# cerbos/cerbos

Measured on NVIDIA H100. Metric: checkresources_decisions_per_sec, higher is better.
Workload: dtype u64

## Files before the change

### cerbos_b200/csrc/cb_core.h

```cpp
#pragma once
#include <stdint.h>
#if !defined(__CUDACC_RTC__)
#include <math.h>
#endif

#include "cerbos_b200_format.h"

#if defined(__CUDACC__)
#define CB_HD __host__ __device__ __forceinline__
#define CB_HD_NOINLINE __host__ __device__ __noinline__
#else
#define CB_HD inline
#define CB_HD_NOINLINE
#endif

namespace cb {

struct alignas(16) U4 { uint32_t x, y, z, w; };

struct TableLayout {
    uint32_t off[CB_IMAGE_SECTIONS];
    uint32_t nV, nRP, nS, nP, nR, nAP, nT, n_slots, n_rows;
    uint32_t has_role_policies, has_parent_roles, has_principal_policies;
    uint32_t image_bytes;
    uint32_t uc_conds_off, uc_rows_off, uc_chain_off, n_uconds;
    uint32_t uc_n_rows;
    uint32_t uc_slots_off;
    uint32_t uc_deny_rows, uc_allow_rows;
    uint32_t theap_words;
    uint32_t uses_runtime;
};

struct TableView {
    const uint8_t *base;
    const TableLayout *L;
    template <typename T>
    CB_HD const T *sec(int id) const { return reinterpret_cast<const T *>(base + L->off[id]); }
    CB_HD const uint32_t *scope_parent() const { return sec<uint32_t>(CB_SEC_SCOPE_PARENT); }
    CB_HD const uint32_t *scope_flags() const { return sec<uint32_t>(CB_SEC_SCOPE_FLAGS); }
    CB_HD const uint32_t *res_block_map() const { return sec<uint32_t>(CB_SEC_RES_BLOCK_MAP); }
    CB_HD const uint8_t *res_exists() const { return sec<uint8_t>(CB_SEC_RES_EXISTS); }
    CB_HD const uint32_t *prin_block_map() const { return sec<uint32_t>(CB_SEC_PRIN_BLOCK_MAP); }
    CB_HD const uint8_t *prin_exists() const { return sec<uint8_t>(CB_SEC_PRIN_EXISTS); }
    CB_HD const uint32_t *prin_of_string() const { return sec<uint32_t>(CB_SEC_PRIN_OF_STRING); }
    CB_HD const cb_block *blocks() const { return sec<cb_block>(CB_SEC_BLOCKS); }
    CB_HD const cb_row *rows() const { return sec<cb_row>(CB_SEC_ROWS); }
    CB_HD const cb_cond *conds() const { return sec<cb_cond>(CB_SEC_CONDS); }
    CB_HD const cb_instr *code() const { return sec<cb_instr>(CB_SEC_CODE); }
    CB_HD const cb_const *consts() const { return sec<cb_const>(CB_SEC_CONSTS); }
    CB_HD const uint64_t *consts_v64() const { return sec<uint64_t>(CB_SEC_CONSTS_V64); }
    CB_HD const uint64_t *theap() const { return sec<uint64_t>(CB_SEC_THEAP); }
    CB_HD const uint32_t *str_off() const { return sec<uint32_t>(CB_SEC_STR_OFF); }
    CB_HD const uint8_t *str_bytes() const { return sec<uint8_t>(CB_SEC_STR_BYTES); }
    CB_HD const uint32_t *par_off() const { return sec<uint32_t>(CB_SEC_ROLE_PARENTS_OFF); }
    CB_HD const uint32_t *par_list() const { return sec<uint32_t>(CB_SEC_ROLE_PARENTS); }
    CB_HD const uint32_t *rp_off() const { return sec<uint32_t>(CB_SEC_ROLEPOL_OFF); }
    CB_HD const cb_rolepol_entry *rp_entries() const { return sec<cb_rolepol_entry>(CB_SEC_ROLEPOL_ENTRIES); }
    CB_HD const cb_rolepol_rule *rp_rules() const { return sec<cb_rolepol_rule>(CB_SEC_ROLEPOL_RULES); }
    CB_HD const uint32_t *rp_apats() const { return sec<uint32_t>(CB_SEC_ROLEPOL_APATS); }
    CB_HD const uint32_t *block_slots_off() const { return sec<uint32_t>(CB_SEC_BLOCK_SLOTS_OFF); }
    CB_HD const uint32_t *block_slots() const { return sec<uint32_t>(CB_SEC_BLOCK_SLOTS); }
    CB_HD const uint32_t *dr_off() const { return sec<uint32_t>(CB_SEC_DR_OFF); }
    CB_HD const uint32_t *dr_entries() const { return sec<uint32_t>(CB_SEC_DR_ENTRIES); }
    CB_HD const uint32_t *dr_parents() const { return sec<uint32_t>(CB_SEC_DR_PARENTS); }
    CB_HD const uint32_t *dr_name_str() const { return sec<uint32_t>(CB_SEC_DR_NAME_STR); }
    CB_HD const uint32_t *row_out() const { return sec<uint32_t>(CB_SEC_ROW_OUT); }
    CB_HD const cb_out_entry *out_entries() const { return sec<cb_out_entry>(CB_SEC_OUT_ENTRIES); }
    CB_HD const cb_cond *uconds() const { return reinterpret_cast<const cb_cond *>(base + L->uc_conds_off); }
    CB_HD const U4 *urows() const { return reinterpret_cast<const U4 *>(base + L->uc_rows_off); }
    CB_HD const uint32_t *uc_slots() const { return reinterpret_cast<const uint32_t *>(base + L->uc_slots_off); }
    CB_HD const U4 *uc_chain() const { return reinterpret_cast<const U4 *>(base + L->uc_chain_off); }
};

enum { CB_MAX_GATHER = 8 };
struct BatchView {
    const cb_hdr0 *hdr0;
    const cb_hdr1 *hdr1;
    const uint32_t *roles;
// ... 4413 lines not shown
    CB_HD UcRowsPacked at(uint32_t first) const { UcRowsPacked r = *this; if (by_slot) r.pk += first; else r.slots += first; return r; }
    CB_HD U4 get(uint32_t ri) const { return ld16(pk + ri); }
    CB_HD U4 slot(uint32_t j) const {
        if (by_slot) return ld16(pk + j);
        const uint32_t ri = ldg(slots + j);
        return uc_slot_record(ld16(pk + (ri != CB_NONE32 ? ri : 0u)), ri != CB_NONE32);
    }
};

struct CachedCols {
    const BatchView *b;
    uint64_t n;
    CB_HD U4 hdr0() const { return ldcol128(b->hdr0 + n); }
    CB_HD uint64_t hdr1() const { return ldcol64(reinterpret_cast<const uint64_t *>(b->hdr1 + n)); }
    CB_HD uint32_t role(uint32_t i) const { return ldcol32(b->roles + (uint64_t)i * b->stride + n); }
    CB_HD uint64_t slot(uint32_t v) const {
#if defined(__CUDA_ARCH__)
        uint64_t x;
        asm("ld.global.nc.u64 %0, [%1];" : "=l"(x) : "l"(b->slots + (uint64_t)v * b->stride + n));
        return x;
#else
        return b->slots[(uint64_t)v * b->stride + n];
#endif
    }
    CB_HD void prefetch_slot(uint32_t) const {}
    CB_HD bool staged() const { return true; }
    CB_HD uint32_t aset_k(uint32_t aset) const { return ldg(b->aset_k + aset); }
    CB_HD const uint64_t *row_am() const { return b->row_am; }
    CB_HD bool stage_result(uint32_t) const { return false; }
};

struct CondWord { uint64_t lo, hi; };
enum { CB_UC_FORM_MASK32 = 0, CB_UC_FORM_MASK64 = 1, CB_UC_FORM_INDEX = 2 };
constexpr uint32_t kUcUnrollRows = 16;
constexpr uint32_t kUcRowsOfLayout = ~0u;
struct GenericConds {
    static constexpr int kForm = CB_UC_FORM_MASK64;
    static constexpr uint32_t kDenyRows = kUcRowsOfLayout, kAllowRows = kUcRowsOfLayout;
    static constexpr uint32_t kListSlots = 0;
    template <typename Cols>
    CB_HD Cols load(const TableView, const BatchView &, const Cols &cols) const { return cols; }
    template <typename Cols>
    CB_HD CondWord operator()(const TableView t, const BatchView &b, const Cols &cols, uint32_t pid, uint64_t n, bool &slow) const {
        if (t.L->n_uconds > 63) { slow = true; CondWord w; w.lo = 1; w.hi = 0; return w; }
        uint64_t val = 1;
        for (uint32_t u = 1, nu = t.L->n_uconds; u <= nu; u++) {
            const U4 cd = ld16(t.uconds() + u);
            uint32_t r;
            if (cd.w) r = flat_dnf_inline(t, b, cols, pid, cd.z, cd.w);
            else r = 4u;
            slow |= (r & 4u) != 0;
            val |= (uint64_t)(r & 1u) << u;
        }
        CondWord w; w.lo = val; w.hi = 0;
        return w;
    }
};

CB_HD uint32_t cond_bit(const CondWord v, uint32_t u) { return (uint32_t)(((u & 64u) ? v.hi : v.lo) >> (u & 63u)) & 1u; }
template <typename RP, int kForm>
CB_HD uint32_t uc_row_pairs(const U4 r, const RP rp, const CondWord v, const uint32_t role_all, const uint32_t shift) {
    const uint32_t vlo = (uint32_t)v.lo, vhi = (uint32_t)(v.lo >> 32);
    const uint32_t miss = kForm == CB_UC_FORM_MASK32   ? r.y & ~vlo
                          : kForm == CB_UC_FORM_MASK64 ? (r.y & ~vlo) | (r.z & ~vhi)
                                                       : (cond_bit(v, r.y & 0xFFu) & cond_bit(v, (r.y >> 8) & 0xFFu)) ^ 1u;
    const uint32_t rc = miss ? 0u : (uint32_t)(rp >> shift) & role_all;
    return r.x * rc;
}
struct UcNoObserver {
    CB_HD void operator()(uint32_t, uint32_t, uint32_t, uint32_t, const CondWord &) const {}
};
template <uint32_t kDenyRows, uint32_t kAllowRows, typename RP, int kForm, typename Rows, typename Obs = UcNoObserver>
CB_HD uint32_t uc_walk(const TableView t, const Rows rows, const RP rp, const CondWord val, const uint32_t r0, const uint32_t bm_base,
                       const uint32_t role_all, uint32_t alive, Obs &&obs = Obs()) {
    constexpr bool kOfLayout = kDenyRows == kUcRowsOfLayout;
    const uint32_t n_deny = kOfLayout ? t.L->uc_deny_rows : kDenyRows, n_allow = kOfLayout ? t.L->uc_allow_rows : kAllowRows;
    const bool segments = n_deny + n_allow != 0;
    uint32_t allow_pairs = 0, level = 0;
    const U4 *chain = t.uc_chain() + bm_base;
    for (uint32_t s = r0; s != CB_NONE32 && alive;) {
        const U4 d = ld16(chain + s);
        uint32_t D = 0, A = 0;
        if (segments) {
            const Rows seg = rows.at(d.x);
            auto slot = [&](uint32_t j) { const U4 r = seg.slot(j); return uc_row_pairs<RP, kForm>(r, rp, val, role_all, r.w); };
#if defined(__CUDA_ARCH__)
#pragma unroll
#endif
            for (uint32_t j = 0; j < n_deny; j++) D |= slot(j);
#if defined(__CUDA_ARCH__)
#pragma unroll
#endif
            for (uint32_t j = 0; j < n_allow; j++) A |= slot(n_deny + j);
            D |= A & d.z;
            A &= d.y;
        } else {
#if defined(__CUDA_ARCH__)
#pragma unroll 4
#endif
            for (uint32_t ri = d.x; ri < d.z; ri++) {
                const U4 r = rows.get(ri);
                const uint32_t p = uc_row_pairs<RP, kForm>(r, rp, val, role_all, r.w & (sizeof(RP) * 8 - 1)), deny = (uint32_t)((int32_t)r.w >> 31);
                D |= p & deny;
                A |= p & ~deny;
            }
        }
        D &= alive;
        alive &= ~D;
        A &= alive;
        allow_pairs |= A;
        alive &= ~A;
        obs(level++, s, D, A, val);
        s = d.w;
    }
    return allow_pairs;
}

template <typename Cols, typename Rows, typename Conds = GenericConds>
// ... 90 lines not shown
    for (uint32_t i = 0; i < RC; i++) {
        const uint32_t rr = cols.role(i);
        gap |= pad && rr != CB_ROLE_PAD;
        pad |= rr == CB_ROLE_PAD;
        n_roles = rr != CB_ROLE_PAD ? i + 1 : n_roles;
        rp |= rr < t.L->nR ? 1ull << (rr * RCP + i) : 0ull;
        req_roles |= rr < t.L->nR ? 1ull << rr : 0ull;
    }
    if (pv != rv || gap) return true;
    const bool lenient = (b.flags & CB_BATCH_FLAG_LENIENT) != 0;
    const uint32_t r0 = chain_start(t, rscope, CB_SCOPE_FLAG_RESOURCE, lenient), p0 = chain_start(t, pscope, CB_SCOPE_FLAG_PRINCIPAL, lenient);
    const uint32_t bm_base = (rv * t.L->nRP + kc) * t.L->nS;
    bool exists = false;
    if (K != 0 && r0 != CB_NONE32 && rv != CB_NONE16 && kc != CB_KIND_NONE) {
        const uint32_t w = ld16(side + bm_base + r0).z;
        if ((w >> 8) > CB_MAX_CHAIN) return true;
        exists = (w & 1u) != 0;
    }
    const bool walk = exists && n_roles != 0;
    const uint32_t role_all = (1u << n_roles) - 1;
    uint32_t allow_pairs = 0, acc = 0;
    uint64_t edr = 0;
    UcMetaObserver ob;
    CondWord val; val.lo = 1; val.hi = 0;
    if (walk) {
        bool slow = false;
        val = conds(t, b, regs, pid, n, slow);
        if (slow) return true;
        const uint32_t amask = K * RC >= 32 ? b.stride_pattern : b.stride_pattern & ((1u << (K * RC)) - 1);
        const uint32_t alive0 = amask * role_all;
        const Rows arows = rows.aset(t, b, aset);
        if ((t.L->nR + 1) * RCP <= 32)
            allow_pairs = uc_walk<Conds::kDenyRows, Conds::kAllowRows, uint32_t, Conds::kForm>(t, arows, (uint32_t)rp | role_all << (t.L->nR * RCP), val, r0, bm_base, role_all, alive0, ob);
        else allow_pairs = uc_walk<Conds::kDenyRows, Conds::kAllowRows, uint64_t, Conds::kForm>(t, arows, rp | (uint64_t)role_all << (t.L->nR * RCP), val, r0, bm_base, role_all, alive0, ob);
        uint32_t need = 0;
        for (uint32_t k = 0; k < K; k++) {
            const uint32_t a = (allow_pairs >> (k * RC)) & role_all, lowest = a & (0u - a);
            need |= (lowest ? lowest | (lowest - 1) : role_all) << (k * RC);
            acc |= (a != 0 ? 1u : 0u) << k;
        }
        const uint32_t undecided = alive0 & ~(allow_pairs | ob.deny), last = ob.levels - 1;
        const uint32_t lv0 = ob.lv0 | ((last & 1u) ? undecided : 0u), lv1 = ob.lv1 | ((last & 2u) ? undecided : 0u), lv2 = ob.lv2 | ((last & 4u) ? undecided : 0u);
        uint32_t top = 0, cand = need;
        if (cand & lv2) { top |= 4u; cand &= lv2; }
        if (cand & lv1) { top |= 2u; cand &= lv1; }
        if (cand & lv0) top |= 1u;
        const U4 *chain = t.uc_chain() + bm_base;
        uint32_t s = r0;
        for (uint32_t l = 0; l <= top && s != CB_NONE32; l++) {
            const U4 m = ld16(side + bm_base + s);
            for (uint32_t e = m.x; e < m.y; e++) {
                const U4 dr = ld16(side + e);
                const bool hit = (dr.y >> 31) != 0 || ((((uint64_t)dr.w << 32) | dr.z) & req_roles) != 0;
                edr |= (uint64_t)(hit && cond_bit(val, dr.y & 0x7FFFFFFFu)) << dr.x;
            }
            s = ld16(chain + s).w;
        }
    }
    store_result(b, cols, n, nullptr, effects, K, acc);
    uint32_t *am = action_meta + n * (uint64_t)KM;
    const uint32_t none = walk ? 0xFFFFu | CB_META_SRC_RESOURCE_POLICY << 16 : 0xFFFFu;
    const U4 *chain = t.uc_chain() + bm_base;
    for (uint32_t k = 0; k < KM; k++) {
        uint32_t w = 0xFFFFu;
        if (k < K) {
            const uint32_t a = (allow_pairs >> (k * RC)) & role_all, d = (ob.deny >> (k * RC)) & role_all, c = a ? a : d;
            w = none;
            if (c) {
                uint32_t s = r0;
                for (uint32_t l = 0, lv = ob.level_of(k * RC + ctz32(c)); l < lv; l++) s = ld16(chain + s).w;
                w = (s & 0xFFFFu) | CB_META_SRC_RESOURCE_POLICY << 16;
            }
        }
        am[k] = w;
    }
    cb_request_meta rm;
    rm.principal_first_scope = (uint16_t)(p0 == CB_NONE32 ? 0xFFFFu : p0);
    rm.resource_first_scope = (uint16_t)(r0 == CB_NONE32 ? 0xFFFFu : r0);
    rm.flags = 0;
    rm.effective_derived_roles = edr;
    req_meta[n] = rm;
    return false;
}

#ifndef CB_LEAN_ONLY
CB_HD_NOINLINE void eval_request_general(const uint8_t *base, const TableLayout *L, const BatchView *b, uint64_t n, uint8_t *bitmap,
                                         uint8_t *effects, uint32_t *status) {
    TableView t; t.base = base; t.L = L;
    eval_request<uint64_t>(t, *b, n, bitmap, effects, status);
}

#endif

}
```

### cerbos_b200/csrc/cb_specialize.h

```cpp
#pragma once
#include <stdint.h>

#include <cstdio>
#include <cstring>
#include <map>
#include <string>
#include <vector>

#include "cerbos_b200_format.h"

namespace cbspec {

struct Limits {
    uint32_t max_shapes = 8;
    uint32_t max_items = 96;
};

inline std::string hex(uint32_t v) {
    char buf[16];
    snprintf(buf, sizeof buf, "0x%xu", v);
    return buf;
}
inline std::string hex64(uint64_t v) {
    char buf[32];
// ... 334 lines not shown
        if (I.op == CB_OP_CONST && i + 1 < code_len) {
            const uint32_t nx = P[i + 1].op;
            if (cond_level(nx)) literal = true;
            if ((nx == CB_OP_JF_KEEP || nx == CB_OP_JT_KEEP) && (e >= code_len || P[i + 1].ic > e)) literal = true;
        }
        if (literal) {
            if (I.ic >= n_consts || consts[4 * I.ic] != CB_T_BOOL) return "";
            st.push_back(consts[4 * I.ic + 2] ? "true" : "false");
            i++;
            continue;
        }
        if (e >= code_len) return "";
        std::vector<uint32_t> key;
        for (uint32_t k = i; k < e; k++) {
            const Ins &J = P[k];
            const bool j = is_jump(J.op);
            key.push_back(J.op | J.ia << 8 | (J.op == CB_OP_TERN ? (J.ib - i) : J.ib) << 16);
            key.push_back(j ? J.ic - i : J.ic);
        }
        auto it = at.ids.find(key);
        if (it == at.ids.end()) {
            if (at.slot_used.size() < n_slots) at.slot_used.resize(n_slots, false);
            uint32_t one = CB_NONE32;
            bool pid = false;
            const std::string body = atom_source(P, i, e, consts, n_consts, n_slots, at.slot_used, &one, &pid);
            if (body.empty()) return "";
            const uint32_t id = (uint32_t)at.src.size();
            at.only_slot.push_back(one);
            at.reads_pid.push_back(pid);
            at.src.push_back("template <typename Cols>\nCB_HD bool uc_atom_" + std::to_string(id) + "(Ctx &c, const Cols &cols) {\n" + body + "}\n");
            it = at.ids.emplace(key, id).first;
        }
        st.push_back("a" + std::to_string(it->second));
        i = e + 1;
    }
    if (!ret || st.size() != 1) return "";
    return st[0];
}

struct UcLimits {
    uint32_t max_terms = 512;
};
struct UcSource {
    std::string src;
    uint32_t n_strpred = 0;
    uint32_t n_atoms = 0;
};
inline UcSource generate_uc(const uint8_t *uc_image, const uint32_t *off, uint32_t uc_conds_off, uint32_t n_uconds, uint32_t n_slots, uint32_t n_consts = 0,
                            const UcLimits lim = UcLimits()) {
    UcSource out;
    if (n_uconds == 0 || n_uconds > 127) return out;
    const uint32_t *const_words = reinterpret_cast<const uint32_t *>(uc_image + off[CB_SEC_CONSTS]);
    Atoms atoms;
    std::vector<std::string> formula(n_uconds + 1);
    const uint32_t *uconds = reinterpret_cast<const uint32_t *>(uc_image + uc_conds_off);
    const uint32_t scope_rows = uconds[0], deny_rows = uconds[1], allow_rows = uconds[2];
    const uint32_t *code = reinterpret_cast<const uint32_t *>(uc_image + off[CB_SEC_CODE]);
    const uint64_t *consts = reinterpret_cast<const uint64_t *>(uc_image + off[CB_SEC_CONSTS_V64]);
    const uint64_t *theap = reinterpret_cast<const uint64_t *>(uc_image + off[CB_SEC_THEAP]);
    const uint32_t kUseMask = ~((uint32_t)(CB_TERM_LIT_F | CB_TERM_GROUP_END) << 8);
    std::map<std::vector<uint32_t>, uint32_t> term_ids;
    std::vector<std::vector<uint32_t>> terms;
    const uint32_t ns = n_slots ? n_slots : 1;
    std::vector<bool> slot_used(ns, false), slot_list(ns, false);
    auto is_slot_kind = [](uint32_t kind) { return kind == CB_OPK_SLOT || kind == CB_OPK_SLOT_ELEM || kind == CB_OPK_SLOT_SIZE; };
    auto use_slot = [&](uint32_t kind, uint32_t v) { if (is_slot_kind(kind) && v < ns) slot_used[v] = true; };
    auto v64_tag = [](uint64_t b) { const uint32_t top = (uint32_t)(b >> 48); return (top & 0xFFF0u) == 0xFFF0u ? (top & 0xFu) : 0u; };
    for (uint32_t u = 1; u <= n_uconds; u++) {
        const uint32_t *cd = uconds + 4 * u;
        if (cd[3] == 0 || ((cd[3] >> 16) & 0xFF) != CB_FLAT_DNF) {
            formula[u] = translate_program(code, cd[0], cd[1], const_words, n_consts, ns, atoms);
            if (formula[u].empty()) return out;
            continue;
        }
        for (uint32_t i = 0, nt = cd[3] & 0xFFFFu; i < nt; i++) {
            const uint32_t *w = code + 2 * (cd[2] + 2 * i);
            std::vector<uint32_t> key = {w[0] & kUseMask, w[1], w[2], w[3]};
            if (term_ids.emplace(key, (uint32_t)terms.size()).second) terms.push_back(key);
        }
    }
    if (terms.size() > lim.max_terms) return out;
    std::vector<char> form(terms.size(), 'G');
    std::vector<uint32_t> pred_of(terms.size(), 0);
    std::vector<uint32_t> pred_terms;
    for (uint32_t q = 0; q < terms.size(); q++) {
        const uint32_t *w = terms[q].data();
        const uint32_t op = w[0] & 0xFF, xk = (w[0] >> 16) & 0xFF, yk = w[0] >> 24;
        switch (op) {
        case CB_TERM_EQ_SS: case CB_TERM_ORD_SS: use_slot(CB_OPK_SLOT, w[1]); use_slot(CB_OPK_SLOT, w[2]); break;
        case CB_TERM_EQ_SC: case CB_TERM_EQ_SP: case CB_TERM_ORD_SC: case CB_TERM_IN_SC: use_slot(CB_OPK_SLOT, w[1]); break;
        case CB_TERM_IN_SS: use_slot(CB_OPK_SLOT, w[1]); use_slot(CB_OPK_SLOT, w[2]); if (w[2] < ns) { slot_list[w[2]] = true; form[q] = 'L'; } break;
        case CB_TERM_IN_CS: use_slot(CB_OPK_SLOT, w[2]); if (w[2] < ns) { slot_list[w[2]] = true; form[q] = 'L'; } break;
        default:
            use_slot(xk, w[1]);
            if (op != CB_TERM_HAS) use_slot(yk, w[2]);
            if (xk == CB_OPK_SLOT_SIZE && w[1] < ns) slot_list[w[1]] = true;
            if (op != CB_TERM_HAS && yk == CB_OPK_SLOT_SIZE && w[2] < ns) slot_list[w[2]] = true;
            if (op == CB_TERM_IN && yk == CB_OPK_SLOT && w[2] < ns) { slot_list[w[2]] = true; form[q] = 'L'; }
            if ((op == CB_TERM_INTERSECTS || op == CB_TERM_SUBSET) && xk == CB_OPK_SLOT && yk == CB_OPK_SLOT && w[1] < ns && w[2] < ns) {
                slot_list[w[1]] = slot_list[w[2]] = true;
                form[q] = 'L';
            }
            if ((op == CB_TERM_STARTS || op == CB_TERM_ENDS || op == CB_TERM_CONTAINS) && xk == CB_OPK_SLOT && yk == CB_OPK_CONST &&
                v64_tag(consts[w[2]]) == CB_V64_STRING && pred_terms.size() < 32) {
                form[q] = 'P';
                pred_of[q] = (uint32_t)pred_terms.size();
                pred_terms.push_back(q);
            }
            break;
        }
    }
    std::vector<int> atom_pred(atoms.src.size(), -1);
    uint32_t n_pred_bits = (uint32_t)pred_terms.size();
    for (uint32_t a = 0; a < atoms.src.size(); a++)
        if (atoms.only_slot[a] != CB_NONE32 && !atoms.reads_pid[a] && n_pred_bits + 2 <= 32) { atom_pred[a] = (int)n_pred_bits; n_pred_bits += 2; }
    std::map<std::pair<uint32_t, uint32_t>, bool> masks;
    std::vector<std::pair<uint32_t, uint32_t>> mask_of(terms.size());
    for (int pass = 0; pass < 2; pass++)
        for (uint32_t q = 0; q < terms.size(); q++) {
            const uint32_t *w = terms[q].data();
            const uint32_t op = w[0] & 0xFF;
// ... 195 lines not shown
            return e;
        }
        case CB_TERM_HAS: return "true";
        case CB_TERM_CMP:
            x = typed_operand(xk, w[1], w[3] & 0xFFFFu, kx); y = typed_operand(yk, w[2], w[3] >> 16, ky);
            if (!kx || !ky) return "";
            if (ci == 0) return kx == ky ? x + " == " + y : "false";
            return kx == 'N' && ky == 'N' ? "typed_ord(" + hex(ci) + ", " + x + ", " + y + ")" : "";
        case CB_TERM_STARTS: case CB_TERM_ENDS: case CB_TERM_CONTAINS:
            x = typed_operand(xk, w[1], w[3] & 0xFFFFu, kx); y = typed_operand(yk, w[2], w[3] >> 16, ky);
            if (kx != 'S' || ky != 'S') return "";
            return "str_tri(t, b, " + std::to_string(op) + "u, typed_box(" + x + "), typed_box(" + y + ")) == TRI_T";
        default: return "";
        }
    };
    std::vector<std::string> tterm(terms.size());
    for (uint32_t q = 0; q < terms.size() && typed; q++) {
        tterm[q] = typed_term(q);
        typed = !tterm[q].empty();
    }
    auto probe_key = [&](const Probe &x) -> std::string {
        const std::string V = std::to_string(x.v);
        if (x.kind == CB_OPK_CONST || x.kind == CB_OPK_PID) return "list_probe_key(" + x.value + ")";
        if (x.kind == CB_OPK_SLOT) return x.v < ns && ty[x.v] == 'S' ? "cols.k" + V : "";
        if (x.kind == CB_OPK_SLOT_ELEM) return "list_elem_key(t, b, cols, " + V + "u, cols.l" + V + ", " + std::to_string(x.aux) + "u)";
        return "";
    };
    for (const auto &pl : probes)
        for (const Probe &x : pl.second) typed &= !probe_key(x).empty();
    std::string s;
    s += "// generated by cb_specialize.h (generate_uc) from the loaded table: every distinct condition, straight-line\n";
    s += "namespace cb {\n";
    for (const std::string &a : atoms.src) s += a;
    auto reg = [&](uint32_t v) { return slot_used[v] || slot_list[v]; };
    s += "struct SpecRegs {\n    CachedCols g;\n";
    for (uint32_t v = 0; v < ns; v++)
        if (reg(v)) s += "    uint64_t s" + std::to_string(v) + ";\n";
    if (typed) {
        s += "    bool typed;   // every slot below holds the type its terms compare it as (SpecConds::load)\n";
        for (uint32_t v = 0; v < ns; v++) {
            const std::string V = std::to_string(v);
            if (ty[v] == 'S') s += "    ListKey k" + V + ";   // string: its probe key (the id when typed)\n";
            if (ty[v] == 'N') s += "    double d" + V + ";\n";
            if (ty[v] == 'B') s += "    bool b" + V + ";\n";
        }
    }
    for (uint32_t v = 0; v < ns; v++)
        if (slot_list[v]) s += "    ListRegs l" + std::to_string(v) + ";\n";
    s += "    CB_HD uint64_t slot(uint32_t v) const {\n        switch (v) {\n";
    for (uint32_t v = 0; v < ns && !typed; v++)
        if (reg(v)) s += "        case " + std::to_string(v) + "u: return s" + std::to_string(v) + ";\n";
    s += "        default: return v < " + std::to_string(ns) + "u ? g.slot(v) : (uint64_t)(CB_V64_BOX_BASE | CB_V64_ERROR) << 48;\n        }\n    }\n};\n";
    s += "struct SpecConds {\n    static constexpr uint32_t n_strpred = " + std::to_string(n_pred_bits) + "u;\n";
    s += std::string("    static constexpr int kForm = ") + (n_uconds <= 31 ? "CB_UC_FORM_MASK32" : n_uconds <= 63 ? "CB_UC_FORM_MASK64" : "CB_UC_FORM_INDEX") + ";   // how the rows name their conditions\n";
    s += "    static constexpr uint32_t kScopeRows = " + std::to_string(scope_rows) + "u;   // rows the walk visits per scope (cb::uc_walk)\n";
    s += "    static constexpr uint32_t kDenyRows = " + std::to_string(deny_rows) + "u, kAllowRows = " + std::to_string(allow_rows) +
         "u;   // segment slots (0 / 0: row ranges)\n";
    s += std::string("    static constexpr bool kPrograms = ") + (have_atoms ? "true" : "false") + ";   // leaf programs: needs the value helpers of cb_core.h\n";
    {
        std::string ls;
        uint32_t nls = 0;
        for (uint32_t v = 0; v < ns && !have_atoms; v++)
            if (slot_list[v]) ls += (nls++ ? ", " : "") + std::to_string(v) + "u";
        s += "    static constexpr uint32_t kListSlots = " + std::to_string(nls) + "u;   // list slots whose headers check_uc_body prefetches\n";
        s += "    static constexpr uint32_t kListSlot[" + std::to_string(nls ? nls : 1u) + "] = {" + (nls ? ls : "0u") + "};\n";
    }
    s += "    template <typename Cols>\n    CB_HD SpecRegs load(const TableView t, const BatchView &b, const Cols &c) const {\n        SpecRegs r;\n        r.g.b = c.b; r.g.n = c.n;\n";
    for (uint32_t v = 0; v < ns; v++)
        if (reg(v)) s += "        r.s" + std::to_string(v) + " = c.slot(" + std::to_string(v) + "u);\n";
    if (typed) {
        std::string guard;
        for (uint32_t v = 0; v < ns; v++) {
            const std::string V = std::to_string(v);
            if (!reg(v)) continue;
            if (ty[v] == 'L') s += "        r.l" + V + " = list_load(t, b, r.s" + V + ");\n";
            if (ty[v] == 'S') s += "        r.k" + V + " = list_probe_key(r.s" + V + ");\n";
            if (ty[v] == 'N') s += "        r.d" + V + " = u2d(r.s" + V + ");\n";
            if (ty[v] == 'B') s += "        r.b" + V + " = (r.s" + V + " & 1u) != 0;\n";
            guard += std::string(guard.empty() ? "" : " & ") + (ty[v] == 'L' ? "typed_list(r.l" + V + ", " + std::to_string(list_need[v]) + "u)"
                                                                 : std::string(ty[v] == 'S' ? "typed_str" : ty[v] == 'N' ? "typed_num" : "typed_bool") + "(r.s" + V + ")");
        }
        s += "        r.typed = " + guard + ";\n";
    } else {
        for (uint32_t v = 0; v < ns; v++)
            if (slot_list[v]) s += "        r.l" + std::to_string(v) + " = list_load(t, b, r.s" + std::to_string(v) + ");\n";
    }
    s += "        return r;\n    }\n";
    s += "    // the predicate word of one string (pre-pass over the string dictionary; bit p = predicate p holds)\n";
    s += "    CB_HD uint32_t strpred(const TableView t, const BatchView &b, uint32_t id) const {\n";
    s += "        OneCols cols; cols.x = ((uint64_t)(CB_V64_BOX_BASE | CB_V64_STRING) << 48) | id;\n        bool slow = false; uint32_t bits = 0u; const uint32_t pid = 0u;\n";
    for (uint32_t p = 0; p < pred_terms.size(); p++) {
        const uint32_t *w = terms[pred_terms[p]].data();
        s += "        bits |= (uint32_t)(term_tri(t, b, cols, pid, U4{" + hex(w[0]) + ", 0x0u, " + hex(w[2]) + ", " + hex(w[3]) + "}, slow) == TRI_T) << " + std::to_string(p) + ";\n";
    }
    {
        bool any = false;
        for (int p : atom_pred) any |= p >= 0;
        if (any) {
            s += "        Ctx c; c.t = &t; c.b = &b; c.req = 0; c.pid = 0; c.edr = 0;\n";
            for (uint32_t a = 0; a < atoms.src.size(); a++)
                if (atom_pred[a] >= 0)
                    s += "        c.unsupported = 0; c.scr_used = 0; bits |= (uint32_t)uc_atom_" + std::to_string(a) + "(c, cols) << " + std::to_string(atom_pred[a]) +
                         "; bits |= (uint32_t)(c.unsupported != 0) << " + std::to_string(atom_pred[a] + 1) + ";\n";
        }
    }
    s += "        (void)slow; (void)pid;\n        return bits;\n    }\n";
    s += "    CB_HD CondWord operator()(const TableView t, const BatchView &b, const SpecRegs &cols, uint32_t pid, uint64_t n, bool &slow) const {\n";
    const std::string in = typed ? "            " : "        ";
    for (const auto &pl : probes) {
        const std::string v = std::to_string(pl.first);
        std::string keys;
        for (uint32_t p = 0; p < pl.second.size(); p++) {
            const std::string xp = "x" + v + "_" + std::to_string(p);
            if (!typed) s += "        const uint64_t " + xp + " = " + pl.second[p].value + ";\n";
            keys += std::string(p ? ", " : "") + (typed ? probe_key(pl.second[p]) : "list_probe_key(" + xp + ")");
        }
        s += "        const ListKey k" + v + "[" + std::to_string(pl.second.size()) + "] = {" + keys + "};\n";
        s += "        const uint32_t h" + v + " = list_probe(cols.l" + v + ", k" + v + ");   // bit p: x" + v + "_p is an element of slot " + v + "\n";
    }
    for (const auto &m : masks) {
        const std::string a = std::to_string(m.first.first), bb = std::to_string(m.first.second);
        s += "        const uint32_t m" + a + "_" + bb + " = list_mask(cols.l" + a + ", cols.l" + bb + ");   // elements of slot " + a + " in slot " + bb + "\n";
    }
    std::string tri;
    if (typed)
        for (const auto &pl : probes)
            for (uint32_t p = 0; p < pl.second.size(); p++)
                tri += in + "const uint64_t x" + std::to_string(pl.first) + "_" + std::to_string(p) + " = " + pl.second[p].value + ";\n";
    for (int list_terms = 1; list_terms >= 0; list_terms--)
        for (uint32_t q = 0; q < terms.size(); q++)
            if ((form[q] == 'L') == (list_terms == 1)) tri += in + "const int q" + std::to_string(q) + " = " + term_code(q) + ";\n";
    std::string atom_src;
    if (have_atoms) {
        atom_src += "        Ctx c; c.t = &t; c.b = &b; c.req = n; c.pid = pid; c.unsupported = 0; c.edr = 0; c.scr_used = 0;\n";
        for (uint32_t a = 0; a < atoms.src.size(); a++) {
            const std::string A = std::to_string(a);
            if (atom_pred[a] >= 0) {
                const std::string P = std::to_string(atom_pred[a]), V = sl(atoms.only_slot[a]);
                atom_src += "        bool a" + A + ";\n        {\n            const uint64_t x = " + V + ";\n            const uint32_t w = v64_tag(x) == CB_V64_STRING && !v64_bad(x) ? ldg(b.strpred + (uint32_t)(x & 0xFFFFFFFFu)) >> " + P + " : 2u;\n";
                atom_src += "            if (w & 2u) { c.scr_used = 0; a" + A + " = uc_atom_" + A + "(c, cols); } else a" + A + " = (w & 1u) != 0;\n        }\n";
            } else {
                atom_src += "        c.scr_used = 0; const bool a" + A + " = uc_atom_" + A + "(c, cols);\n";
            }
        }
        atom_src += "        slow |= c.unsupported != 0;   // a value the device forms cannot hold: the general kernel reports it\n";
    } else atom_src += "        (void)n;\n";
    std::string typed_src;
    std::vector<std::string> cond_src(n_uconds + 1);
    if (typed) {
        typed_src += "        if (uc_typed(cols.typed)) {   // every term a plain boolean: no error, no deferral\n";
        for (uint32_t q = 0; q < terms.size(); q++) typed_src += "            const bool t" + std::to_string(q) + " = " + tterm[q] + ";\n";
    }
    for (uint32_t u = 1; u <= n_uconds; u++) {
        const uint32_t *cd = uconds + 4 * u;
        const std::string word = u < 64 ? "val.lo" : "val.hi", sh = std::to_string(u & 63u);
        if (!formula[u].empty()) {
            cond_src[u] = "        " + word + " |= (uint64_t)(" + formula[u] + ") << " + sh + ";   // distinct condition " + std::to_string(u) + " (program)\n";
            continue;
        }
        const uint32_t nt = cd[3] & 0xFFFFu, negate = (cd[3] >> 24) & 1u;
        std::string &c = cond_src[u];
        c += in + "{   // distinct condition " + std::to_string(u) + "\n" + in + "    bool any = false, group = true;\n";
        std::string any, group;
        for (uint32_t i = 0; i < nt; i++) {
            const uint32_t *w = code + 2 * (cd[2] + 2 * i);
            const uint32_t flags = (w[0] >> 8) & 0xFFu;
            const uint32_t q = term_ids[{w[0] & kUseMask, w[1], w[2], w[3]}];
            c += in + "    group &= term_lit(q" + std::to_string(q) + ", " + hex(flags) + ");\n";
            group += std::string(group.empty() ? "" : " & ") + (flags & CB_TERM_LIT_F ? "!t" : "t") + std::to_string(q);
            if (flags & CB_TERM_GROUP_END) {
                c += in + "    any |= group; group = true;\n";
                any += std::string(any.empty() ? "" : " | ") + "(" + group + ")";
                group.clear();
            }
        }
        c += in + "    " + word + std::string(" |= (uint64_t)(any != ") + (negate ? "true" : "false") + ") << " + sh + ";\n" + in + "}\n";
        if (any.empty()) any = "false";
        typed_src += "            " + word + " |= (uint64_t)(" + (negate ? "!(" + any + ")" : any) + ") << " + sh + ";   // condition " + std::to_string(u) + "\n";
    }
    if (typed) {
        s += atom_src + "        CondWord val; val.lo = 1ull; val.hi = 0ull;\n" + typed_src + "        } else {   // the tri-state terms on the slot words, reloaded (cols.slot)\n" + tri;
        for (uint32_t u = 1; u <= n_uconds; u++) if (formula[u].empty()) s += cond_src[u];
        s += "        }\n";
        for (uint32_t u = 1; u <= n_uconds; u++) if (!formula[u].empty()) s += cond_src[u];
    } else {
        s += tri + atom_src + "        CondWord val; val.lo = 1ull; val.hi = 0ull;\n";
        for (uint32_t u = 1; u <= n_uconds; u++) s += cond_src[u];
    }
    s += "        return val;\n    }\n};\n}  // namespace cb\n";
    out.src = s;
    out.n_strpred = n_pred_bits;
    out.n_atoms = (uint32_t)atoms.src.size();
    return out;
}

}
```

### cerbos_b200/csrc/cb_uc.h

```cpp
#pragma once
#include <stdint.h>

#include <cstring>
#include <map>
#include <string>
#include <tuple>
#include <vector>

#include "cb_core.h"

namespace cbuc {

constexpr uint32_t kMaxUconds = 127;
constexpr uint32_t kMaxMaskUconds = 63;

struct Image {
    bool ok = false;
    std::string why;
    std::vector<uint8_t> bytes;
    cb::TableLayout lay{};
    uint32_t n_uconds = 0, n_flat = 0;
    bool needs_spec() const { return n_flat != n_uconds || n_uconds > kMaxMaskUconds; }
    uint32_t scope_rows = 0;
    uint32_t deny_rows = 0, allow_rows = 0;
    uint32_t n_gids = 0, n_gids_flat = 0;
    std::vector<uint32_t> ucond_of_gid;
};

inline Image build(const uint8_t *image, const uint32_t *off, const uint64_t *len, const uint32_t *meta, const cb::TableLayout &lay) {
    Image out;
    const uint32_t n_blocks = meta[CB_META_N_BLOCKS], n_rows = meta[CB_META_N_ROWS], n_conds = meta[CB_META_N_CONDS];
    if (n_blocks == 0) { out.why = "no policy blocks"; return out; }
    if (lay.nR > 64) { out.why = "more than 64 roles"; return out; }
    const uint32_t *blocks = reinterpret_cast<const uint32_t *>(image + off[CB_SEC_BLOCKS]);
    const uint32_t *rows = reinterpret_cast<const uint32_t *>(image + off[CB_SEC_ROWS]);
    const uint32_t *conds = reinterpret_cast<const uint32_t *>(image + off[CB_SEC_CONDS]);
    if (len[CB_SEC_BLOCKS] < (uint64_t)n_blocks * 16 || len[CB_SEC_ROWS] < (uint64_t)n_rows * 16 || len[CB_SEC_CONDS] < (uint64_t)n_conds * 16) {
        out.why = "section sizes do not match META";
        return out;
    }
    std::map<std::tuple<uint32_t, uint32_t, uint32_t>, uint32_t> ids;
    std::vector<uint32_t> ucond_rec;
    ucond_rec.assign(4, 0);
    out.ucond_of_gid.assign(n_conds, 0);
    for (uint32_t g = 0; g < n_conds; g++) {
        const uint32_t *cd = conds + 4 * g;
        const bool flat = cd[3] != 0 && ((cd[3] >> 16) & 0xFF) == CB_FLAT_DNF;
        const auto key = flat ? std::make_tuple(1u, cd[2], cd[3]) : std::make_tuple(0u, cd[0], cd[1]);
        auto it = ids.find(key);
        if (it == ids.end()) {
            const uint32_t u = (uint32_t)ids.size() + 1;
            if (u > kMaxUconds) { out.why = "more than 127 distinct conditions"; return out; }
            it = ids.emplace(key, u).first;
            ucond_rec.insert(ucond_rec.end(), {cd[0], cd[1], flat ? cd[2] : 0u, flat ? cd[3] : 0u});
            out.n_flat += flat;
        }
        out.ucond_of_gid[g] = it->second;
        out.n_gids++;
        out.n_gids_flat += flat;
    }
    out.n_uconds = (uint32_t)ids.size();
    std::vector<uint32_t> urows(4 * (size_t)(n_rows ? n_rows : 1), 0);
    std::vector<uint32_t> ublocks(blocks, blocks + 4 * (size_t)n_blocks);
    const bool index_form = out.n_uconds > kMaxMaskUconds;
    for (uint32_t b = 0; b < n_blocks; b++) {
        const uint32_t *bl = blocks + 4 * b;
        if ((uint64_t)bl[0] + bl[1] > n_rows || (uint64_t)bl[2] + bl[3] > n_conds) { out.why = "block out of range"; return out; }
        uint32_t at = bl[0], n_deny = 0;
        for (int pass = 0; pass < 2; pass++) {
            for (uint32_t r = 0; r < bl[1]; r++) {
                const uint32_t *row = rows + 4 * (bl[0] + r);
                const uint32_t role = row[0] & 0xFFFFu, c = row[0] >> 16, dc = row[1] & 0xFFFFu, effect = row[2] & 0xFFu;
                if ((effect == CB_EFFECT_DENY) != (pass == 0)) continue;
                if ((c && c > bl[3]) || (dc && dc > bl[3])) { out.why = "row condition out of range"; return out; }
                if (role != CB_ROLE_ANY && role >= 64) { out.why = "role id out of range"; return out; }
                const uint32_t uc = c ? out.ucond_of_gid[bl[2] + c - 1] : 0, udc = dc ? out.ucond_of_gid[bl[2] + dc - 1] : 0;
                const uint64_t need = index_form ? 0ull : (1ull | 1ull << uc | 1ull << udc);
                uint32_t *u = urows.data() + 4 * (size_t)at++;
                u[0] = bl[0] + r;
                u[1] = (role == CB_ROLE_ANY ? 0xFFu : role) | effect << 8;
                u[2] = index_form ? (uc | udc << 8) : (uint32_t)need;
                u[3] = index_form ? 0u : (uint32_t)(need >> 32);
                n_deny += pass == 0;
            }
        }
        ublocks[4 * b + 2] = n_deny;
        ublocks[4 * b + 3] = 0;
    }
    const uint32_t nS = meta[CB_META_N_SCOPES];
    const uint64_t n_map = (uint64_t)meta[CB_META_N_VERSIONS] * meta[CB_META_N_RESPATS] * nS;
    if (nS == 0 || len[CB_SEC_SCOPE_PARENT] < (uint64_t)nS * 4 || len[CB_SEC_SCOPE_FLAGS] < (uint64_t)nS * 4 || len[CB_SEC_RES_BLOCK_MAP] < n_map * 4) {
        out.why = "scope tables do not match the block map";
        return out;
    }
    const uint32_t *parent = reinterpret_cast<const uint32_t *>(image + off[CB_SEC_SCOPE_PARENT]);
    const uint32_t *sflags = reinterpret_cast<const uint32_t *>(image + off[CB_SEC_SCOPE_FLAGS]);
    const uint32_t *bmap = reinterpret_cast<const uint32_t *>(image + off[CB_SEC_RES_BLOCK_MAP]);
    std::vector<uint32_t> next(nS);
    for (uint32_t s = 0; s < nS; s++) {
        uint32_t x = s, steps = 0;
        do { x = parent[x]; } while (x != CB_NONE32 && x < nS && ++steps <= nS && !(sflags[x] & CB_SCOPE_FLAG_RESOURCE));
        if (x != CB_NONE32 && (x >= nS || steps > nS)) { out.why = "scope parent chain out of range"; return out; }
        next[s] = x;
    }
    std::vector<uint8_t> used(n_blocks, 0);
    for (uint64_t e = 0; e < n_map; e++) {
        const uint32_t bid = bmap[e];
        if (bid == CB_NONE32) continue;
        if (bid >= n_blocks) { out.why = "block map entry out of range"; return out; }
        used[bid] |= 1 | (((sflags[e % nS] >> CB_SCOPE_PERM_SHIFT) & 3) == 1) << 1;
    }
    uint32_t max_deny = 0, max_allow = 0, max_deny_only = 0;
    for (uint32_t b = 0; b < n_blocks; b++) {
        const uint32_t *bl = ublocks.data() + 4 * (size_t)b;
        if (used[b] & 2) {
            max_deny = bl[2] > max_deny ? bl[2] : max_deny;
            max_allow = bl[1] - bl[2] > max_allow ? bl[1] - bl[2] : max_allow;
        } else if (used[b]) max_deny_only = bl[2] > max_deny_only ? bl[2] : max_deny_only;
    }
    if (max_deny_only > max_deny + max_allow) max_allow = max_deny_only - max_deny;
    const uint32_t seg = max_deny + max_allow;
    const bool segments = seg >= 1 && seg <= cb::kUcUnrollRows && ((uint64_t)n_blocks + 1) * seg < (1ull << 31);
    std::vector<uint32_t> slots;
    if (segments) {
        out.deny_rows = max_deny;
        out.allow_rows = max_allow;
        slots.assign(((size_t)n_blocks + 1) * seg, CB_NONE32);
        for (uint32_t b = 0; b < n_blocks; b++) {
            const uint32_t *bl = ublocks.data() + 4 * (size_t)b;
            const uint32_t n_use = (used[b] & 2) ? bl[1] : used[b] ? bl[2] : 0;
            for (uint32_t r = 0; r < n_use; r++)
                slots[(size_t)(b + 1) * seg + (r < bl[2] || !(used[b] & 2) ? r : max_deny + r - bl[2])] = bl[0] + r;
        }
    }
    std::vector<uint32_t> chain(4 * (size_t)n_map, 0);
    for (uint64_t e = 0; e < n_map; e++) {
        const uint32_t s = (uint32_t)(e % nS), bid = bmap[e];
        uint32_t *d = chain.data() + 4 * e;
        if (bid != CB_NONE32) {
            const uint32_t *bl = ublocks.data() + 4 * (size_t)bid;
            const bool allow_counts = ((sflags[s] >> CB_SCOPE_PERM_SHIFT) & 3) == 1;
            if (segments) {
                d[0] = (bid + 1) * seg;
                d[1] = allow_counts ? ~0u : 0u;
                d[2] = (used[bid] & 2) ? 0u : ~0u;
            } else {
                d[0] = bl[0];
                d[1] = bl[0] + bl[2];
                d[2] = allow_counts ? bl[0] + bl[1] : d[1];
                out.scope_rows = d[2] - d[0] > out.scope_rows ? d[2] - d[0] : out.scope_rows;
            }
        }
        d[3] = next[s];
    }
    if (segments) out.scope_rows = seg;
    ucond_rec[0] = out.scope_rows;
    ucond_rec[1] = out.deny_rows;
    ucond_rec[2] = out.allow_rows;
    out.lay = lay;
    for (auto &o : out.lay.off) o = 0;
    auto append = [&](const void *p, uint64_t n) {
        const uint32_t at = (uint32_t)out.bytes.size();
        out.bytes.resize((out.bytes.size() + n + 15) & ~(size_t)15, 0);
        if (n) memcpy(out.bytes.data() + at, p, n);
        return at;
    };
    append("CBUC", 4);
    for (int id : {CB_SEC_SCOPE_PARENT, CB_SEC_SCOPE_FLAGS, CB_SEC_CODE, CB_SEC_CONSTS, CB_SEC_CONSTS_V64, CB_SEC_THEAP,
                   CB_SEC_STR_OFF, CB_SEC_STR_BYTES})
        out.lay.off[id] = append(image + off[id], len[id]);
    out.lay.uc_conds_off = append(ucond_rec.data(), ucond_rec.size() * 4);
    out.lay.uc_rows_off = append(urows.data(), urows.size() * 4);
    out.lay.uc_chain_off = append(chain.data(), chain.size() * 4);
    out.lay.uc_slots_off = segments ? append(slots.data(), slots.size() * 4) : 0;
    out.lay.n_uconds = out.n_uconds;
    out.lay.uc_n_rows = segments ? (uint32_t)slots.size() : (uint32_t)(urows.size() / 4);
    out.lay.uc_deny_rows = out.deny_rows;
    out.lay.uc_allow_rows = out.allow_rows;
    out.lay.theap_words = (uint32_t)(len[CB_SEC_THEAP] / 8);
    out.lay.image_bytes = (uint32_t)out.bytes.size();
    out.ok = true;
    return out;
}

struct MetaSide {
    bool ok = false;
    std::string why;
    std::vector<uint32_t> words;
};

inline MetaSide build_meta(const uint8_t *image, const uint32_t *off, const uint64_t *len, const uint32_t *meta, const cb::TableLayout &lay, const Image &uc) {
    MetaSide out;
    if (!uc.ok) { out.why = "no unique-condition image"; return out; }
    if (lay.has_principal_policies || lay.has_role_policies || lay.has_parent_roles || lay.uses_runtime) {
        out.why = "principal / role policies, parent roles or runtime.effectiveDerivedRoles";
        return out;
    }
    const uint32_t nS = lay.nS, n_blocks = meta[CB_META_N_BLOCKS];
    const uint64_t n_map = (uint64_t)lay.nV * lay.nRP * nS;
    const uint8_t *pex = image + off[CB_SEC_PRIN_EXISTS];
    for (uint64_t i = 0; i < (uint64_t)lay.nV * nS; i++)
        if (pex[i]) { out.why = "principal-policy existence bits"; return out; }
    const uint32_t *bmap = reinterpret_cast<const uint32_t *>(image + off[CB_SEC_RES_BLOCK_MAP]);
    const uint8_t *rex = image + off[CB_SEC_RES_EXISTS];
    const uint32_t *dr_off = reinterpret_cast<const uint32_t *>(image + off[CB_SEC_DR_OFF]);
    const uint32_t *dr_ent = reinterpret_cast<const uint32_t *>(image + off[CB_SEC_DR_ENTRIES]);
    const uint32_t *dr_par = reinterpret_cast<const uint32_t *>(image + off[CB_SEC_DR_PARENTS]);
    const uint64_t n_ent = len[CB_SEC_DR_ENTRIES] / 16, n_par = len[CB_SEC_DR_PARENTS] / 4;
    const uint32_t *chain = reinterpret_cast<const uint32_t *>(uc.bytes.data() + uc.lay.uc_chain_off);
    std::vector<uint32_t> levels(nS, 0);
    for (uint32_t s = 0; s < nS; s++) {
        uint32_t n = 0;
        for (uint32_t x = s; x != CB_NONE32 && n <= CB_MAX_CHAIN; x = chain[4 * (uint64_t)x + 3]) n++;
        levels[s] = n;
    }
    out.words.assign(4 * n_map, 0);
    std::vector<uint32_t> first(n_blocks, CB_NONE32), end(n_blocks, 0);
    for (uint64_t e = 0; e < n_map; e++) {
        const uint32_t s = (uint32_t)(e % nS), bid = bmap[e];
        uint32_t exists = 0;
        for (uint32_t x = s, n = 0; x != CB_NONE32 && n <= CB_MAX_CHAIN; x = chain[4 * (e - s + x) + 3], n++) exists |= rex[e - s + x] & CB_EXISTS_RESOURCE_KIND;
        out.words[4 * e + 2] = (exists ? 1u : 0u) | levels[s] << 8;
        if (bid == CB_NONE32) continue;
        if (first[bid] == CB_NONE32) {
            first[bid] = (uint32_t)(out.words.size() / 4);
            if (dr_off[bid] > dr_off[bid + 1] || dr_off[bid + 1] > n_ent) { out.why = "derived-role range out of range"; return out; }
            for (uint32_t j = dr_off[bid]; j < dr_off[bid + 1]; j++) {
                const uint32_t *en = dr_ent + 4 * (uint64_t)j;
                if ((uint64_t)en[2] + en[3] > n_par || (en[1] && en[1] - 1 >= uc.ucond_of_gid.size())) { out.why = "derived-role entry out of range"; return out; }
                uint64_t mask = 0;
                bool any = false;
                for (uint32_t q = 0; q < en[3]; q++) {
                    const uint32_t pr = dr_par[en[2] + q];
                    if (pr == CB_ROLE_ANY) any = true;
                    else if (pr < lay.nR) mask |= 1ull << pr;
                }
                const uint32_t u = en[1] ? uc.ucond_of_gid[en[1] - 1] : 0u;
                out.words.insert(out.words.end(), {en[0] & 63u, u | (any ? 1u << 31 : 0u), (uint32_t)mask, (uint32_t)(mask >> 32)});
            }
            end[bid] = (uint32_t)(out.words.size() / 4);
        }
        out.words[4 * e] = first[bid];
        out.words[4 * e + 1] = end[bid];
    }
    out.ok = true;
    return out;
}

}
```

Measured before the change: 94.64 billion.

## Fold negated conditions onto shared base bits with complement masks

Distinct conditions that differ only by negation now share one evaluated base bit, and rows carry a need-false mask alongside the need-true mask. The goal is fewer condition evaluations per request, and often a narrower mask form (32-bit instead of 64-bit or index form). In exchange the row miss test gets an extra mask, the image layout and derived-role side table change, and the generated specialised code changes.

```diff
diff --git a/cerbos_b200/csrc/cb_core.h b/cerbos_b200/csrc/cb_core.h
--- a/cerbos_b200/csrc/cb_core.h
+++ b/cerbos_b200/csrc/cb_core.h
@@ -24,6 +24,7 @@
     uint32_t has_role_policies, has_parent_roles, has_principal_policies;
     uint32_t image_bytes;
     uint32_t uc_conds_off, uc_rows_off, uc_chain_off, n_uconds;
+    uint32_t uc_complement;
     uint32_t uc_n_rows;
     uint32_t uc_slots_off;
     uint32_t uc_deny_rows, uc_allow_rows;
@@ -4543,18 +4544,18 @@
             slow |= (r & 4u) != 0;
             val |= (uint64_t)(r & 1u) << u;
         }
-        CondWord w; w.lo = val; w.hi = 0;
+        CondWord w; w.lo = t.L->uc_complement ? val | (uint64_t)~(uint32_t)val << 32 : val; w.hi = 0;
         return w;
     }
 };
 
-CB_HD uint32_t cond_bit(const CondWord v, uint32_t u) { return (uint32_t)(((u & 64u) ? v.hi : v.lo) >> (u & 63u)) & 1u; }
+CB_HD uint32_t cond_bit(const CondWord v, uint32_t u, uint32_t neg) { return ((uint32_t)(((u & 64u) ? v.hi : v.lo) >> (u & 63u)) & 1u) ^ neg; }
 template <typename RP, int kForm>
 CB_HD uint32_t uc_row_pairs(const U4 r, const RP rp, const CondWord v, const uint32_t role_all, const uint32_t shift) {
     const uint32_t vlo = (uint32_t)v.lo, vhi = (uint32_t)(v.lo >> 32);
-    const uint32_t miss = kForm == CB_UC_FORM_MASK32   ? r.y & ~vlo
+    const uint32_t miss = kForm == CB_UC_FORM_MASK32   ? (r.y & ~vlo) | (r.z & vlo)
                           : kForm == CB_UC_FORM_MASK64 ? (r.y & ~vlo) | (r.z & ~vhi)
-                                                       : (cond_bit(v, r.y & 0xFFu) & cond_bit(v, (r.y >> 8) & 0xFFu)) ^ 1u;
+                                                       : (cond_bit(v, r.y & 0xFFu, 0u) & cond_bit(v, (r.y >> 8) & 0xFFu, 0u)) ^ 1u;
     const uint32_t rc = miss ? 0u : (uint32_t)(rp >> shift) & role_all;
     return r.x * rc;
 }
@@ -4751,7 +4752,7 @@
             for (uint32_t e = m.x; e < m.y; e++) {
                 const U4 dr = ld16(side + e);
                 const bool hit = (dr.y >> 31) != 0 || ((((uint64_t)dr.w << 32) | dr.z) & req_roles) != 0;
-                edr |= (uint64_t)(hit && cond_bit(val, dr.y & 0x7FFFFFFFu)) << dr.x;
+                edr |= (uint64_t)(hit && cond_bit(val, dr.y & 0x3FFFFFFFu, (dr.y >> 30) & 1u)) << dr.x;
             }
             s = ld16(chain + s).w;
         }
diff --git a/cerbos_b200/csrc/cb_specialize.h b/cerbos_b200/csrc/cb_specialize.h
--- a/cerbos_b200/csrc/cb_specialize.h
+++ b/cerbos_b200/csrc/cb_specialize.h
@@ -410,9 +410,11 @@
     if (n_uconds == 0 || n_uconds > 127) return out;
     const uint32_t *const_words = reinterpret_cast<const uint32_t *>(uc_image + off[CB_SEC_CONSTS]);
     Atoms atoms;
-    std::vector<std::string> formula(n_uconds + 1);
     const uint32_t *uconds = reinterpret_cast<const uint32_t *>(uc_image + uc_conds_off);
     const uint32_t scope_rows = uconds[0], deny_rows = uconds[1], allow_rows = uconds[2];
+    const uint32_t n_bits = uconds[3] ? uconds[3] : n_uconds;
+    const uint32_t *base_of = uconds[3] ? uconds + 4 * (n_bits + 1) : nullptr;
+    std::vector<std::string> formula(n_bits + 1);
     const uint32_t *code = reinterpret_cast<const uint32_t *>(uc_image + off[CB_SEC_CODE]);
     const uint64_t *consts = reinterpret_cast<const uint64_t *>(uc_image + off[CB_SEC_CONSTS_V64]);
     const uint64_t *theap = reinterpret_cast<const uint64_t *>(uc_image + off[CB_SEC_THEAP]);
@@ -424,7 +426,7 @@
     auto is_slot_kind = [](uint32_t kind) { return kind == CB_OPK_SLOT || kind == CB_OPK_SLOT_ELEM || kind == CB_OPK_SLOT_SIZE; };
     auto use_slot = [&](uint32_t kind, uint32_t v) { if (is_slot_kind(kind) && v < ns) slot_used[v] = true; };
     auto v64_tag = [](uint64_t b) { const uint32_t top = (uint32_t)(b >> 48); return (top & 0xFFF0u) == 0xFFF0u ? (top & 0xFu) : 0u; };
-    for (uint32_t u = 1; u <= n_uconds; u++) {
+    for (uint32_t u = 1; u <= n_bits; u++) {
         const uint32_t *cd = uconds + 4 * u;
         if (cd[3] == 0 || ((cd[3] >> 16) & 0xFF) != CB_FLAT_DNF) {
             formula[u] = translate_program(code, cd[0], cd[1], const_words, n_consts, ns, atoms);
@@ -726,7 +728,12 @@
         if (reg(v)) s += "        case " + std::to_string(v) + "u: return s" + std::to_string(v) + ";\n";
     s += "        default: return v < " + std::to_string(ns) + "u ? g.slot(v) : (uint64_t)(CB_V64_BOX_BASE | CB_V64_ERROR) << 48;\n        }\n    }\n};\n";
     s += "struct SpecConds {\n    static constexpr uint32_t n_strpred = " + std::to_string(n_pred_bits) + "u;\n";
-    s += std::string("    static constexpr int kForm = ") + (n_uconds <= 31 ? "CB_UC_FORM_MASK32" : n_uconds <= 63 ? "CB_UC_FORM_MASK64" : "CB_UC_FORM_INDEX") + ";   // how the rows name their conditions\n";
+    s += std::string("    static constexpr int kForm = ") + (n_bits <= 31 ? "CB_UC_FORM_MASK32" : n_bits <= 63 ? "CB_UC_FORM_MASK64" : "CB_UC_FORM_INDEX") + ";   // how the rows name their conditions\n";
+    if (base_of) {
+        s += "    // " + std::to_string(n_uconds) + " distinct conditions on " + std::to_string(n_bits) + " base conditions, one bit each:\n";
+        for (uint32_t d = 0; d < n_uconds; d++)
+            s += "    // distinct condition " + std::to_string(d + 1) + ": " + (base_of[d] >> 31 ? "!" : "") + "base condition " + std::to_string(base_of[d] & 0x7FFFFFFFu) + "\n";
+    }
     s += "    static constexpr uint32_t kScopeRows = " + std::to_string(scope_rows) + "u;   // rows the walk visits per scope (cb::uc_walk)\n";
     s += "    static constexpr uint32_t kDenyRows = " + std::to_string(deny_rows) + "u, kAllowRows = " + std::to_string(allow_rows) +
          "u;   // segment slots (0 / 0: row ranges)\n";
@@ -820,21 +827,22 @@
         atom_src += "        slow |= c.unsupported != 0;   // a value the device forms cannot hold: the general kernel reports it\n";
     } else atom_src += "        (void)n;\n";
     std::string typed_src;
-    std::vector<std::string> cond_src(n_uconds + 1);
+    std::vector<std::string> cond_src(n_bits + 1);
+    const std::string what = base_of ? "base condition " : "distinct condition ", cast = n_bits <= 31 ? "(uint32_t)" : "(uint64_t)";
     if (typed) {
         typed_src += "        if (uc_typed(cols.typed)) {   // every term a plain boolean: no error, no deferral\n";
         for (uint32_t q = 0; q < terms.size(); q++) typed_src += "            const bool t" + std::to_string(q) + " = " + tterm[q] + ";\n";
     }
-    for (uint32_t u = 1; u <= n_uconds; u++) {
+    for (uint32_t u = 1; u <= n_bits; u++) {
         const uint32_t *cd = uconds + 4 * u;
         const std::string word = u < 64 ? "val.lo" : "val.hi", sh = std::to_string(u & 63u);
         if (!formula[u].empty()) {
-            cond_src[u] = "        " + word + " |= (uint64_t)(" + formula[u] + ") << " + sh + ";   // distinct condition " + std::to_string(u) + " (program)\n";
+            cond_src[u] = "        " + word + " |= " + cast + "(" + formula[u] + ") << " + sh + ";   // " + what + std::to_string(u) + " (program)\n";
             continue;
         }
         const uint32_t nt = cd[3] & 0xFFFFu, negate = (cd[3] >> 24) & 1u;
         std::string &c = cond_src[u];
-        c += in + "{   // distinct condition " + std::to_string(u) + "\n" + in + "    bool any = false, group = true;\n";
+        c += in + "{   // " + what + std::to_string(u) + "\n" + in + "    bool any = false, group = true;\n";
         std::string any, group;
         for (uint32_t i = 0; i < nt; i++) {
             const uint32_t *w = code + 2 * (cd[2] + 2 * i);
@@ -848,18 +856,18 @@
                 group.clear();
             }
         }
-        c += in + "    " + word + std::string(" |= (uint64_t)(any != ") + (negate ? "true" : "false") + ") << " + sh + ";\n" + in + "}\n";
+        c += in + "    " + word + " |= " + cast + "(any != " + (negate ? "true" : "false") + ") << " + sh + ";\n" + in + "}\n";
         if (any.empty()) any = "false";
-        typed_src += "            " + word + " |= (uint64_t)(" + (negate ? "!(" + any + ")" : any) + ") << " + sh + ";   // condition " + std::to_string(u) + "\n";
+        typed_src += "            " + word + " |= " + cast + "(" + (negate ? "!(" + any + ")" : any) + ") << " + sh + ";   // " + (base_of ? what : std::string("condition ")) + std::to_string(u) + "\n";
     }
     if (typed) {
         s += atom_src + "        CondWord val; val.lo = 1ull; val.hi = 0ull;\n" + typed_src + "        } else {   // the tri-state terms on the slot words, reloaded (cols.slot)\n" + tri;
-        for (uint32_t u = 1; u <= n_uconds; u++) if (formula[u].empty()) s += cond_src[u];
+        for (uint32_t u = 1; u <= n_bits; u++) if (formula[u].empty()) s += cond_src[u];
         s += "        }\n";
-        for (uint32_t u = 1; u <= n_uconds; u++) if (!formula[u].empty()) s += cond_src[u];
+        for (uint32_t u = 1; u <= n_bits; u++) if (!formula[u].empty()) s += cond_src[u];
     } else {
         s += tri + atom_src + "        CondWord val; val.lo = 1ull; val.hi = 0ull;\n";
-        for (uint32_t u = 1; u <= n_uconds; u++) s += cond_src[u];
+        for (uint32_t u = 1; u <= n_bits; u++) s += cond_src[u];
     }
     s += "        return val;\n    }\n};\n}  // namespace cb\n";
     out.src = s;
diff --git a/cerbos_b200/csrc/cb_uc.h b/cerbos_b200/csrc/cb_uc.h
--- a/cerbos_b200/csrc/cb_uc.h
+++ b/cerbos_b200/csrc/cb_uc.h
@@ -13,6 +13,8 @@
 
 constexpr uint32_t kMaxUconds = 127;
 constexpr uint32_t kMaxMaskUconds = 63;
+constexpr uint32_t kMaxComplementBits = 31;
+constexpr uint32_t kNegated = 1u << 31;
 
 struct Image {
     bool ok = false;
@@ -20,7 +22,9 @@
     std::vector<uint8_t> bytes;
     cb::TableLayout lay{};
     uint32_t n_uconds = 0, n_flat = 0;
-    bool needs_spec() const { return n_flat != n_uconds || n_uconds > kMaxMaskUconds; }
+    uint32_t n_bits = 0;
+    bool complement = false;
+    bool needs_spec() const { return n_flat != n_uconds || n_bits > kMaxMaskUconds; }
     uint32_t scope_rows = 0;
     uint32_t deny_rows = 0, allow_rows = 0;
     uint32_t n_gids = 0, n_gids_flat = 0;
@@ -39,10 +43,10 @@
         out.why = "section sizes do not match META";
         return out;
     }
-    std::map<std::tuple<uint32_t, uint32_t, uint32_t>, uint32_t> ids;
-    std::vector<uint32_t> ucond_rec;
-    ucond_rec.assign(4, 0);
-    out.ucond_of_gid.assign(n_conds, 0);
+    std::map<std::tuple<uint32_t, uint32_t, uint32_t>, uint32_t> ids, base_ids;
+    std::vector<uint32_t> rec_distinct, rec_base;
+    std::vector<uint32_t> ucond_of, base_of;
+    ucond_of.assign(n_conds, 0);
     for (uint32_t g = 0; g < n_conds; g++) {
         const uint32_t *cd = conds + 4 * g;
         const bool flat = cd[3] != 0 && ((cd[3] >> 16) & 0xFF) == CB_FLAT_DNF;
@@ -52,17 +56,33 @@
             const uint32_t u = (uint32_t)ids.size() + 1;
             if (u > kMaxUconds) { out.why = "more than 127 distinct conditions"; return out; }
             it = ids.emplace(key, u).first;
-            ucond_rec.insert(ucond_rec.end(), {cd[0], cd[1], flat ? cd[2] : 0u, flat ? cd[3] : 0u});
+            rec_distinct.insert(rec_distinct.end(), {cd[0], cd[1], flat ? cd[2] : 0u, flat ? cd[3] : 0u});
             out.n_flat += flat;
-        }
-        out.ucond_of_gid[g] = it->second;
+            const uint32_t neg = flat ? cd[3] & 1u << 24 : 0u;
+            const auto bkey = flat ? std::make_tuple(1u, cd[2], cd[3] & ~neg) : key;
+            auto bt = base_ids.find(bkey);
+            if (bt == base_ids.end()) {
+                bt = base_ids.emplace(bkey, (uint32_t)base_ids.size() + 1).first;
+                rec_base.insert(rec_base.end(), {cd[0], cd[1], flat ? cd[2] : 0u, flat ? cd[3] & ~neg : 0u});
+            }
+            base_of.push_back(bt->second | (neg ? kNegated : 0u));
+        }
+        ucond_of[g] = it->second;
         out.n_gids++;
         out.n_gids_flat += flat;
     }
     out.n_uconds = (uint32_t)ids.size();
+    out.complement = base_ids.size() < ids.size() && base_ids.size() <= kMaxComplementBits;
+    out.n_bits = out.complement ? (uint32_t)base_ids.size() : out.n_uconds;
+    out.ucond_of_gid.assign(n_conds, 0);
+    for (uint32_t g = 0; g < n_conds; g++) out.ucond_of_gid[g] = out.complement ? base_of[ucond_of[g] - 1] : ucond_of[g];
+    std::vector<uint32_t> ucond_rec(4, 0);
+    const std::vector<uint32_t> &recs = out.complement ? rec_base : rec_distinct;
+    ucond_rec.insert(ucond_rec.end(), recs.begin(), recs.end());
+    if (out.complement) ucond_rec.insert(ucond_rec.end(), base_of.begin(), base_of.end());
     std::vector<uint32_t> urows(4 * (size_t)(n_rows ? n_rows : 1), 0);
     std::vector<uint32_t> ublocks(blocks, blocks + 4 * (size_t)n_blocks);
-    const bool index_form = out.n_uconds > kMaxMaskUconds;
+    const bool index_form = out.n_bits > kMaxMaskUconds;
     for (uint32_t b = 0; b < n_blocks; b++) {
         const uint32_t *bl = blocks + 4 * b;
         if ((uint64_t)bl[0] + bl[1] > n_rows || (uint64_t)bl[2] + bl[3] > n_conds) { out.why = "block out of range"; return out; }
@@ -75,12 +95,14 @@
                 if ((c && c > bl[3]) || (dc && dc > bl[3])) { out.why = "row condition out of range"; return out; }
                 if (role != CB_ROLE_ANY && role >= 64) { out.why = "role id out of range"; return out; }
                 const uint32_t uc = c ? out.ucond_of_gid[bl[2] + c - 1] : 0, udc = dc ? out.ucond_of_gid[bl[2] + dc - 1] : 0;
-                const uint64_t need = index_form ? 0ull : (1ull | 1ull << uc | 1ull << udc);
+                uint64_t need = 1, need_false = 0;
+                for (const uint32_t x : {uc, udc})
+                    if (!index_form) (x & kNegated ? need_false : need) |= 1ull << (x & ~kNegated);
                 uint32_t *u = urows.data() + 4 * (size_t)at++;
                 u[0] = bl[0] + r;
                 u[1] = (role == CB_ROLE_ANY ? 0xFFu : role) | effect << 8;
                 u[2] = index_form ? (uc | udc << 8) : (uint32_t)need;
-                u[3] = index_form ? 0u : (uint32_t)(need >> 32);
+                u[3] = index_form ? 0u : out.complement ? (uint32_t)need_false : (uint32_t)(need >> 32);
                 n_deny += pass == 0;
             }
         }
@@ -157,6 +179,7 @@
     ucond_rec[0] = out.scope_rows;
     ucond_rec[1] = out.deny_rows;
     ucond_rec[2] = out.allow_rows;
+    ucond_rec[3] = out.complement ? out.n_bits : 0u;
     out.lay = lay;
     for (auto &o : out.lay.off) o = 0;
     auto append = [&](const void *p, uint64_t n) {
@@ -173,7 +196,8 @@
     out.lay.uc_rows_off = append(urows.data(), urows.size() * 4);
     out.lay.uc_chain_off = append(chain.data(), chain.size() * 4);
     out.lay.uc_slots_off = segments ? append(slots.data(), slots.size() * 4) : 0;
-    out.lay.n_uconds = out.n_uconds;
+    out.lay.n_uconds = out.n_bits;
+    out.lay.uc_complement = out.complement;
     out.lay.uc_n_rows = segments ? (uint32_t)slots.size() : (uint32_t)(urows.size() / 4);
     out.lay.uc_deny_rows = out.deny_rows;
     out.lay.uc_allow_rows = out.allow_rows;
@@ -236,7 +260,8 @@
                     else if (pr < lay.nR) mask |= 1ull << pr;
                 }
                 const uint32_t u = en[1] ? uc.ucond_of_gid[en[1] - 1] : 0u;
-                out.words.insert(out.words.end(), {en[0] & 63u, u | (any ? 1u << 31 : 0u), (uint32_t)mask, (uint32_t)(mask >> 32)});
+                out.words.insert(out.words.end(), {en[0] & 63u, (u & ~kNegated) | (u & kNegated ? 1u << 30 : 0u) | (any ? 1u << 31 : 0u),
+                                                   (uint32_t)mask, (uint32_t)(mask >> 32)});
             }
             end[bid] = (uint32_t)(out.words.size() / 4);
         }
```

After: 99.13 billion, median of 6. +4.7%, better.
